# nameofuser1/vad

Hardware: AMD Instinct MI355X
Metric: MFCC+FFN frames/sec on 16 kHz 25 ms/10 ms hop (higher is better)
Workload: dtype f32; 1 GPU; C3/C4: MFCC + FFN VAD forward, 1 clip of F frames per GPU (25 ms frames, 10 ms hop, 512-pt FFT, 26 mel, 13 MFCC, analyser 5-frame features), labels gathered to rank 0; frames_per_gpu=1000000, ffn=13-64-64-2, hip_streams=2, parallelism=clip-shard x1

## Files before the change

### vad_amd/csrc/ffn_kernel.hip

```cpp
#include "vad_common.h"
#include "features.h"
#include "ffn_dev.h"

namespace vad {

enum Src { kFromMfcc = 0, kFromRows = 1 };

template <int KS0, int T1, int T2, int T3, int T4, int NC, int SRC>
__global__ __launch_bounds__(256) void ffn_kernel(FfnDev net, const float* __restrict__ in,
                                                  int64_t n_rows, int mfcc_n, int mode,
                                                  uint8_t* __restrict__ labels) {
  using TP = Topo<KS0, T1, T2, T3, T4, NC>;
  const int lane = threadIdx.x & 63;
  const int g = lane >> 4;
  const int jw = lane & 15;
  const int in_dim = net.dims[0];

  float fa[TP::NA];
  float fb[TP::NB];
  float fv[TP::NV + TP::NVB + 1];
  load_frags<TP>(net.frag, lane, fa, fb, fv);

  const int64_t n_tiles = (n_rows + 15) / 16;
  const int64_t wave_id = (int64_t)blockIdx.x * (blockDim.x >> 6) + (threadIdx.x >> 6);
  const int64_t n_waves = (int64_t)gridDim.x * (blockDim.x >> 6);
  for (int64_t tile = wave_id; tile < n_tiles; tile += n_waves) {
    const int64_t w = tile * 16 + jw;
    const bool valid = w < n_rows;
    float x[KS0];
#pragma unroll
    for (int s = 0; s < KS0; ++s) {
      const int f = 4 * s + g;
      float v = 0.f;
      if (f < in_dim && valid) {
        if constexpr (SRC == kFromMfcc) {
          const float* r0 = in + w * mfcc_n;
          v = window_feature(r0, r0 + mfcc_n, r0 + 2 * mfcc_n, r0 + 3 * mfcc_n, r0 + 4 * mfcc_n,
                             f, mfcc_n, mode);
        } else {
          v = in[w * in_dim + f];
        }
      }
      x[s] = v;
    }
    const f32x4 z = mlp_forward<KS0, T1, T2, T3, T4, NC>(fa, fb, fv, x);
    if (g == 0 && valid) {
      labels[w] = (uint8_t)argmax_classes(z, net.n_classes);
      store_logits(net.logits, w, z, net.n_classes);
    }
  }
}

#ifndef VAD_FFN_WIN_PRIO
#define VAD_FFN_WIN_PRIO 1
#endif
constexpr int kChunk = 64;
constexpr int kXStride = 68;

template <int KS0, int T1, int T2, int T3, int T4, int NC, int MN, bool H3, int MODE = -1>
__device__ __forceinline__ void ffn_window_body(const FfnDev& net, const float* __restrict__ mfcc,
                                                int64_t n_rows, int mfcc_n_rt, int mode_rt,
                                                uint8_t* __restrict__ labels) {
  const int mode = MODE >= 0 ? MODE : mode_rt;
  using TP = Topo<KS0, T1, T2, T3, T4, NC>;
  using HP = HTopo<TP, KS0, T1, T2, T3, T4>;
  static_assert(!H3 || (MN > 0 && MN * (kChunk / 4) <= 256), "split-f16 needs the sliding feature phase");
  __shared__ float rows[2][(kChunk + 4) * kMaxCoefs];
  __shared__ __attribute__((aligned(16))) float X[2][kChunk * kXStride];
  __shared__ int wnan[2][kChunk];
  const int mfcc_n = MN > 0 ? MN : mfcc_n_rt;
  const int tid = threadIdx.x;
  const int lane = tid & 63;
  const int wv = tid >> 6;
  const int g = lane >> 4;
  const int jw = lane & 15;
  const int in_dim = net.dims[0];
  const int nfeat = 3 * mfcc_n;

  constexpr int kNA = H3 ? 1 : TP::NA;
  constexpr int kNH = H3 ? HP::NS : 1;
  float fa[kNA];
  float fb[TP::NB];
  float fv[TP::NV + TP::NVB + 1];
  u4 fh[kNH][2];
  if constexpr (H3) {
    load_frags<TP, true>(net.frag, lane, fa, fb, fv);
    load_fragh<HP>(net.fragh, lane, fh);
    for (int i = tid; i < 2 * kChunk * kXStride; i += 256) (&X[0][0])[i] = 0.f;
  } else {
    load_frags<TP>(net.frag, lane, fa, fb, fv);
  }

  const int64_t n_frames = n_rows + 5;
  const int64_t n_chunks = (n_rows + kChunk - 1) / kChunk;
  constexpr int kRowRegs = ((kChunk + 4) * kMaxCoefs + 255) / 256;
  float pre[2][kRowRegs];
  constexpr int kPackRegs = MN > 0 ? ((kChunk + 4) * MN + 255) / 256 : 1;
  static_assert(MN == 0 || 256 * kPackRegs <= (kChunk + 4) * kMaxCoefs, "packed rows overflow");
  auto load_rows = [&](int64_t ch, float (&dst)[kRowRegs]) {
    const int64_t base = ch * kChunk;
    const int64_t avail = ch < n_chunks ? n_frames - base : 0;
    const int nr = (int)(avail < kChunk + 4 ? avail : kChunk + 4);
    if constexpr (MN > 0) {
#pragma unroll
      for (int q = 0; q < kPackRegs; ++q) {
        const int i = tid + 256 * q;
        const bool ok = i < nr * MN;
        const float v = mfcc[ok ? base * MN + i : 0];
        dst[q] = ok ? v : 0.f;
      }
    } else {
#pragma unroll
      for (int q = 0; q < kRowRegs; ++q) {
        const int i = tid + 256 * q;
        dst[q] = i < nr * mfcc_n ? mfcc[base * mfcc_n + i] : 0.f;
      }
    }
  };
  load_rows(blockIdx.x, pre[0]);
  load_rows(blockIdx.x + gridDim.x, pre[1]);
  int buf = 0;
  for (int64_t ch = blockIdx.x; ch < n_chunks; ch += gridDim.x, buf ^= 1) {
    const int64_t base = ch * kChunk;
    float* rw_ = rows[buf];
    float* Xb = X[buf];
    if constexpr (MN > 0) {
#pragma unroll
      for (int q = 0; q < kPackRegs; ++q) {
        rw_[tid + 256 * q] = pre[0][q];
        pre[0][q] = pre[1][q];
      }
    } else {
#pragma unroll
      for (int q = 0; q < kRowRegs; ++q) {
        const int i = tid + 256 * q;
        if (i < (kChunk + 4) * mfcc_n) {
          const int r = i / mfcc_n, c = i - r * mfcc_n;
          rw_[r * kMaxCoefs + c] = pre[0][q];
        }
        pre[0][q] = pre[1][q];
      }
    }
    if (H3 && tid < kChunk) wnan[buf][tid] = 0;
    __syncthreads();
    load_rows(ch + 2 * (int64_t)gridDim.x, pre[1]);
    const int64_t nwin64 = n_rows - base;
    const int nwin = (int)(nwin64 < kChunk ? nwin64 : kChunk);
    if constexpr (MN > 0 && MN * (kChunk / 4) <= 256) {
      const int c = tid % MN, q = tid / MN;
      if (q < kChunk / 4) {
        float a[8];
#pragma unroll
        for (int k = 0; k < 8; ++k) a[k] = rw_[(4 * q + k) * MN + c];
        const bool m0 = !H3 || c < in_dim, m1 = !H3 || MN + c < in_dim, m2 = !H3 || 2 * MN + c < in_dim;
        constexpr bool kD1 = !H3 || MN < 4 * KS0, kD2 = !H3 || 2 * MN < 4 * KS0;
#pragma unroll
        for (int k = 0; k < 4; ++k) {
          const Feat3 ft = feature_triple(a[k], a[k + 1], a[k + 2], a[k + 3], a[k + 4], mode);
          float* xw = Xb + (4 * q + k) * kXStride;
          if constexpr (H3) {
            const bool nan = (m0 || (kD2 && m2)) && ft.mn != ft.mn;
            __hip_atomic_fetch_or(&wnan[buf][4 * q + k], (int)nan, __ATOMIC_RELAXED,
                                  __HIP_MEMORY_SCOPE_WORKGROUP);
            xw[c] = m0 && !nan ? ft.mn : 0.f;
            if constexpr (kD1) xw[MN + c] = m1 ? ft.d1 : 0.f;
            if constexpr (kD2) xw[2 * MN + c] = m2 && !nan ? ft.d2 : 0.f;
          } else {
            xw[c] = ft.mn;
            xw[MN + c] = ft.d1;
            xw[2 * MN + c] = ft.d2;
          }
        }
      }
    } else
    for (int i = tid; i < nwin * mfcc_n; i += 256) {
      const int w = i / mfcc_n, c = i - w * mfcc_n;
      constexpr int kRS = MN > 0 ? MN : kMaxCoefs;
      const float* r = rw_ + w * kRS + c;
      const Feat3 ft = feature_triple(r[0], r[kRS], r[2 * kRS], r[3 * kRS], r[4 * kRS], mode);
      float* xw = Xb + w * kXStride;
      if constexpr (H3) {
        xw[c] = c < in_dim ? ft.mn : 0.f;
        xw[mfcc_n + c] = mfcc_n + c < in_dim ? ft.d1 : 0.f;
        xw[2 * mfcc_n + c] = 2 * mfcc_n + c < in_dim ? ft.d2 : 0.f;
      } else {
        xw[c] = ft.mn;
        xw[mfcc_n + c] = ft.d1;
        xw[2 * mfcc_n + c] = ft.d2;
      }
    }
    __syncthreads();
    const int wl = wv * 16 + jw;
    const int64_t w = base + wl;
#if VAD_FFN_WIN_PRIO
    __builtin_amdgcn_sched_barrier(0);
    __builtin_amdgcn_s_setprio(VAD_FFN_WIN_PRIO);
    __builtin_amdgcn_sched_barrier(0);
#endif
    f32x4 z;
    if constexpr (H3) {
      float x0[HP::K0][8];
      constexpr bool M0 = kMerge0<KS0>;
      const v4f* xr = reinterpret_cast<const v4f*>(Xb + wl * kXStride + 8 * (M0 ? (g & 1) : g));
#pragma unroll
      for (int s = 0; s < HP::K0; ++s) {
        const v4f lo4 = xr[8 * s], hi4 = xr[8 * s + 1];
#pragma unroll
        for (int q = 0; q < 4; ++q) {
          x0[s][q] = lo4[q];
          x0[s][q + 4] = hi4[q];
        }
      }
      if constexpr (M0) {
#pragma unroll
        for (int q = 0; q < 8; ++q)
          if (8 + q >= 13) x0[0][q] = 8 * (g & 1) + q < 13 ? x0[0][q] : 0.f;
      }
      z = mlp_forward_h3<KS0, T1, T2, T3, T4, NC>(FragRegs{fh}, (const float*)fb, (const float*)fv, x0);
      if (wnan[buf][wl]) z = (f32x4){__builtin_nanf(""), __builtin_nanf(""), __builtin_nanf(""), __builtin_nanf("")};
    } else {
      float x[KS0];
#pragma unroll
      for (int s = 0; s < KS0; ++s) {
        const int f = 4 * s + g;
        x[s] = (f < in_dim && f < nfeat && wl < nwin) ? Xb[wl * kXStride + f] : 0.f;
      }
      z = mlp_forward<KS0, T1, T2, T3, T4, NC>(fa, fb, fv, x);
    }
#if VAD_FFN_WIN_PRIO
    __builtin_amdgcn_sched_barrier(0);
    __builtin_amdgcn_s_setprio(0);
    __builtin_amdgcn_sched_barrier(0);
#endif
    if (g == 0 && wl < nwin) {
      labels[w] = (uint8_t)argmax_classes(z, net.n_classes);
      store_logits(net.logits, w, z, net.n_classes);
    }
  }
}

template <int KS0, int T1, int T2, int T3, int T4, int NC, int MN>
__global__ __launch_bounds__(256) void ffn_window_kernel(FfnDev net, const float* __restrict__ mfcc,
                                                         int64_t n_rows, int mfcc_n_rt, int mode,
                                                         uint8_t* __restrict__ labels) {
  ffn_window_body<KS0, T1, T2, T3, T4, NC, MN, false>(net, mfcc, n_rows, mfcc_n_rt, mode, labels);
}

template <int KS0, int T1, int T2, int T3, int T4, int NC, int MN, int MODE>
__global__ __launch_bounds__(256) __attribute__((amdgpu_waves_per_eu(2))) void ffn_window_h3_kernel(
    FfnDev net, const float* __restrict__ mfcc, int64_t n_rows, int mfcc_n_rt, int mode,
    uint8_t* __restrict__ labels) {
  ffn_window_body<KS0, T1, T2, T3, T4, NC, MN, true, MODE>(net, mfcc, n_rows, mfcc_n_rt, mode, labels);
}

#ifndef VAD_FFN_WAVE
#define VAD_FFN_WAVE 1
#endif
#ifndef VAD_FFN_PF
#define VAD_FFN_PF 2
#endif
#ifndef VAD_FFN_WAVE_MFMA_OUT
#define VAD_FFN_WAVE_MFMA_OUT 0
#endif
#ifndef VAD_FFN_LDS_SLOTS
#define VAD_FFN_LDS_SLOTS 1
#endif
#ifndef VAD_FFN_ALL_LDS
#define VAD_FFN_ALL_LDS 1
#endif
template <int KS0, int NC>
struct WaveResidency {
  static constexpr bool kAll = VAD_FFN_ALL_LDS != 0 && KS0 == 4 && NC <= 2;
  static constexpr bool kLdsFrags = KS0 == 10 || NC > 2 || kAll;
  static constexpr bool kLdsSlots = (VAD_FFN_LDS_SLOTS != 0 && !kLdsFrags) || kAll;
#ifndef VAD_FFN_ALL_WPS
#define VAD_FFN_ALL_WPS 4
#endif
  static constexpr int kWavesPerSimd = kAll ? VAD_FFN_ALL_WPS : KS0 == 10 ? 3 : kLdsSlots ? 3 : 2;
};
template <int LO_FROM>
struct FragSplitRes {
  const u4 (*p)[2];
  const u4* lo;
  int base;
  __device__ u4 get(int sl, int h) const {
    return (h == 1 && base + sl >= LO_FROM) ? lo[(base + sl - LO_FROM) * 64] : p[sl][h];
  }
  __device__ FragSplitRes at(int off) const { return {p + off, lo, base + off}; }
};
struct LdsRow {
  const float* p;
  __device__ float operator[](int s) const { return p[s]; }
  __device__ LdsRow operator+(int off) const { return {p + off}; }
};
constexpr int kWRows = (kWTile + 4) * 13;
constexpr int kWRowRegs = (kWRows + 63) / 64;

#ifndef VAD_FFN_WPB
#define VAD_FFN_WPB 4
#endif
constexpr int kWpb = VAD_FFN_WPB;
template <int KS0, int T1, int T2, int T3, int T4, int NC, int MODE, bool LG>
__global__ __launch_bounds__(64 * kWpb) __attribute__((amdgpu_waves_per_eu(WaveResidency<KS0, NC>::kWavesPerSimd))) void ffn_wave_kernel(
    FfnDev net, const float* __restrict__ mfcc, int64_t n_rows, uint8_t* __restrict__ labels) {
  using TP = Topo<KS0, T1, T2, T3, T4, NC, VAD_FFN_WAVE_MFMA_OUT != 0>;
  using HP = HTopo<TP, KS0, T1, T2, T3, T4>;
  constexpr int MN = 13;
  static_assert(KS0 == 4 || KS0 == 10, "specialised topologies: 13 or 39 inputs");
  constexpr int IN = KS0 == 4 ? MN : 3 * MN;
  constexpr int XS = 32 * HP::K0 + 4;
  __shared__ float rows_s[kWpb][kWRows];
  __shared__ __attribute__((aligned(16))) float x_s[kWpb][kWTile * XS];
  __shared__ int flat_s[kWpb][kWTile];
  const int lane = threadIdx.x & 63;
  const int wv = __builtin_amdgcn_readfirstlane(threadIdx.x >> 6);
  const int g = lane >> 4;
  const int jw = lane & 15;
  float* R = rows_s[wv];
  float* X = x_s[wv];
  int* FL = flat_s[wv];

  constexpr bool kLdsFrags = WaveResidency<KS0, NC>::kLdsFrags;
  constexpr bool kLdsSlots = WaveResidency<KS0, NC>::kLdsSlots;
  constexpr int NSL = TP::NB + TP::NV + TP::NVB;
  constexpr bool kDiff = NC == 2 && TP::VL && TP::NL == 3 && kLdsSlots;
  constexpr int NSD = kDiff ? TP::TIL * 4 + 1 : 0;
  constexpr int NSLP = (NSL + NSD + 3) & ~3;
  __shared__ __attribute__((aligned(16))) float slot_s[kLdsSlots ? 4 * NSLP : 1];
#ifndef VAD_FFN_PRIO
#define VAD_FFN_PRIO 3
#endif
#ifndef VAD_FFN_PRIO_FEAT
#define VAD_FFN_PRIO_FEAT 0
#endif
#ifndef VAD_FFN_LO_ALL
#define VAD_FFN_LO_ALL 1
#endif
  constexpr int kLoFrom = VAD_FFN_LO_ALL ? 0 : HP::S0;
  constexpr int kLoSlots = kLdsSlots && !kLdsFrags ? HP::NS - kLoFrom : 0;
  __shared__ u4 fhlo_s[kLoSlots > 0 ? kLoSlots * 64 : 1];
  float fa[1];
  float fb[kLdsSlots ? 1 : TP::NB];
  float fv[kLdsSlots ? 1 : TP::NV + TP::NVB + 1];
  if constexpr (kLdsSlots) {
    auto slot_val = [&](int sl, int gg) {
      const int src_sl = sl < TP::NB ? TP::NA_ALL + sl
                                     : TP::NA_ALL + TP::NB + (sl - TP::NB < TP::NV ? sl - TP::NB
                                                                                  : 4 * TP::TIL * 4 + sl - TP::NB - TP::NV);
      return net.frag[src_sl * 64 + 16 * gg];
    };
    for (int i = threadIdx.x; i < 4 * NSLP; i += 64 * kWpb) {
      const int gg = i / NSLP, sl = i - gg * NSLP;
      float v = 0.f;
      if (sl < NSL) {
        v = slot_val(sl, gg);
      } else if (sl < NSL + NSD) {
        const int q = sl - NSL;
        v = q < TP::TIL * 4 ? slot_val(TP::NB + TP::TIL * 4 + q, gg) - slot_val(TP::NB + q, gg)
                            : slot_val(TP::NB + TP::NV + 1, gg) - slot_val(TP::NB + TP::NV, gg);
      }
      slot_s[i] = v;
    }
    for (int i = threadIdx.x; i < kLoSlots * 64; i += 64 * kWpb)
      fhlo_s[i] = reinterpret_cast<const u4*>(net.fragh)[(2 * (kLoFrom + i / 64) + 1) * 64 + (i & 63)];
    __syncthreads();
  } else {
    load_frags<TP, true>(net.frag, lane, fa, fb, fv);
  }
  const auto fbs = [&] {
    if constexpr (kLdsSlots) return LdsRow{slot_s + g * NSLP};
    else return (const float*)fb;
  }();
  const auto fvs = [&] {
    if constexpr (kLdsSlots) return LdsRow{slot_s + g * NSLP + TP::NB};
    else return (const float*)fv;
  }();
  __shared__ u4 fh_s[kLdsFrags ? HP::NS * 2 * 64 : 1];
  u4 fh_r[kLdsFrags ? 1 : HP::NS][2];
  if constexpr (kLdsFrags) {
    for (int i = threadIdx.x; i < HP::NS * 2 * 64; i += 64 * kWpb) fh_s[i] = reinterpret_cast<const u4*>(net.fragh)[i];
    __syncthreads();
  } else {
    load_fragh<HP>(net.fragh, lane, *reinterpret_cast<u4(*)[HP::NS][2]>(fh_r));
  }
  const auto fh = [&] {
    if constexpr (kLdsFrags) return FragLds{fh_s, lane};
    else if constexpr (kLdsSlots) return FragSplitRes<kLoFrom>{fh_r, fhlo_s + lane, 0};
    else return FragRegs{fh_r};
  }();
  for (int i = lane; i < kWTile * XS; i += 64) X[i] = 0.f;

  const int64_t n_tiles = (n_rows + kWTile - 1) / kWTile;
  const int64_t total = (n_rows + 4) * MN;
  const int64_t wave_id = (int64_t)blockIdx.x * kWpb + wv;
  const int64_t n_waves = (int64_t)gridDim.x * kWpb;
  auto load = [&](int64_t t, float (&dst)[kWRowRegs]) {
    const int64_t base = t * (kWTile * MN);
    const float* tb = mfcc + base;
    const int64_t rem = total - 1 - base;
    const unsigned limb = 4u * (unsigned)(rem < kWRows ? rem : kWRows);
#pragma unroll
    for (int q = 0; q < kWRowRegs; ++q) {
      const unsigned ob = 4u * (unsigned)(lane + 64 * q);
      dst[q] = *reinterpret_cast<const float*>(reinterpret_cast<const char*>(tb) + (ob < limb ? ob : limb));
    }
  };
  __builtin_amdgcn_s_waitcnt(0x0f70);
  auto tile_body = [&](int64_t t, int64_t tn, float (&pre)[kWRowRegs]) {
    wave_lds_handoff();
#pragma unroll
    for (int q = 0; q < kWRowRegs; ++q)
      if (lane + 64 * q < kWRows) R[lane + 64 * q] = pre[q];
    load(tn < n_tiles ? tn : t, pre);
#if VAD_FFN_PRIO_FEAT
    __builtin_amdgcn_sched_barrier(0);
    __builtin_amdgcn_s_setprio(VAD_FFN_PRIO_FEAT);
    __builtin_amdgcn_sched_barrier(0);
#endif
    wave_tile_features<IN, XS, MODE>(R, X, FL, lane);
#if VAD_FFN_PRIO || VAD_FFN_PRIO_FEAT
    __builtin_amdgcn_sched_barrier(0);
    __builtin_amdgcn_s_setprio(VAD_FFN_PRIO);
    __builtin_amdgcn_sched_barrier(0);
#endif
    f32x4 z;
    int lab;
    if constexpr (kDiff) {
      lab = wave_tile_label2<KS0, T1, T2, IN, XS, false, wave_tile_in_bounded<MODE, IN>>(
          X, FL, lane, fh, fbs, fvs, LdsRow{slot_s + g * NSLP + NSL}, net.h1_bounded, LG ? &z : nullptr);
    } else {
      lab = wave_tile_classify<KS0, T1, T2, T3, T4, NC, VAD_FFN_WAVE_MFMA_OUT != 0, IN, XS, false,
                               wave_tile_in_bounded<MODE, IN>>(X, FL, lane, fh, fbs, fvs, net.n_classes, z);
    }
#if VAD_FFN_PRIO && !VAD_FFN_PRIO_FEAT
    __builtin_amdgcn_sched_barrier(0);
    __builtin_amdgcn_s_setprio(0);
    __builtin_amdgcn_sched_barrier(0);
#endif
    const int64_t w = t * kWTile + jw;
    if (g == 0 && w < n_rows) {
      labels[w] = (uint8_t)lab;
      if constexpr (LG) store_logits(net.logits, w, z, net.n_classes);
    }
  };
#ifndef VAD_FFN_PF_ALL
#define VAD_FFN_PF_ALL 1
#endif
  constexpr int kPF = WaveResidency<KS0, NC>::kAll ? VAD_FFN_PF_ALL : VAD_FFN_PF;
  float pre[kPF][kWRowRegs];
#pragma unroll
  for (int k = 0; k < kPF; ++k) {
    const int64_t tk = wave_id + k * n_waves;
    load(tk < n_tiles ? tk : 0, pre[k]);
  }
  for (int64_t t = wave_id; t < n_tiles; t += kPF * n_waves) {
#pragma unroll
    for (int k = 0; k < kPF; ++k) {
      const int64_t tk = t + k * n_waves;
      if (k > 0 && tk >= n_tiles) break;
      tile_body(tk, tk + kPF * n_waves, pre[k]);
    }
  }
}

#ifndef VAD_FFN_GROUP
#define VAD_FFN_GROUP 2
#endif
#ifndef VAD_FFN_GROUP_WPS
#define VAD_FFN_GROUP_WPS 0
#endif
template <int NT>
constexpr int kGroupWps = VAD_FFN_GROUP_WPS ? VAD_FFN_GROUP_WPS : NT <= 2 ? 4 : 2;
#ifndef VAD_FFN_GROUP_WPB
#define VAD_FFN_GROUP_WPB 8
#endif
constexpr int kGWpb = VAD_FFN_GROUP_WPB;
template <int MODE, int NT>
__global__ __launch_bounds__(64 * kGWpb) __attribute__((amdgpu_waves_per_eu(kGroupWps<NT>))) void ffn_wave_group_kernel(
    FfnDev net, const float* __restrict__ mfcc, int64_t n_rows, uint8_t* __restrict__ labels) {
  constexpr int KS0 = 4, T1 = 4, T2 = 4, NC = 2, MN = 13, IN = 13, XS = 20;
  using TP = Topo<KS0, T1, T2, 1, 0, NC, false>;
  using HP = HTopo<TP, KS0, T1, T2, 1, 0>;
  static_assert(TP::VL && TP::NL == 3, "VALU output layer");
  __shared__ float rows_s[kGWpb][NT][kWRows];
  __shared__ __attribute__((aligned(16))) float x_s[kGWpb][NT][kWTile * XS];
  __shared__ int flat_s[kGWpb][NT][kWTile];
  constexpr int NSL = TP::NB + TP::NV + TP::NVB;
  constexpr int NSD = TP::TIL * 4 + 1;
  constexpr int NSLP = (NSL + NSD + 3) & ~3;
  __shared__ __attribute__((aligned(16))) float slot_s[4 * NSLP];
  __shared__ u4 fh_s[HP::NS * 2 * 64];
  const int lane = threadIdx.x & 63;
  const int wv = __builtin_amdgcn_readfirstlane(threadIdx.x >> 6);
  const int g = lane >> 4;
  const int jw = lane & 15;
  const int64_t n_tiles = (n_rows + kWTile - 1) / kWTile;
  const int64_t total = (n_rows + 4) * MN;
  const int64_t wave_id = (int64_t)blockIdx.x * kGWpb + wv;
  const int64_t n_waves = (int64_t)gridDim.x * kGWpb;
  auto load = [&](int64_t t, float (&dst)[kWRowRegs]) {
    const int64_t base = t * (kWTile * MN);
    const float* tb = mfcc + base;
    const int64_t rem = total - 1 - base;
    const unsigned limb = 4u * (unsigned)(rem < kWRows ? rem : kWRows);
#pragma unroll
    for (int q = 0; q < kWRowRegs; ++q) {
      const unsigned ob = 4u * (unsigned)(lane + 64 * q);
      dst[q] = *reinterpret_cast<const float*>(reinterpret_cast<const char*>(tb) + (ob < limb ? ob : limb));
    }
  };
  auto member = [&](int64_t t, int k) { return t + k * n_waves < n_tiles ? t + k * n_waves : t; };
  float pre[NT][kWRowRegs];
  if (wave_id < n_tiles) {
#pragma unroll
    for (int k = 0; k < NT; ++k) load(member(wave_id, k), pre[k]);
  }
  {
    auto slot_val = [&](int sl, int gg) {
      const int src_sl = sl < TP::NB ? TP::NA_ALL + sl
                                     : TP::NA_ALL + TP::NB + (sl - TP::NB < TP::NV ? sl - TP::NB
                                                                                  : 4 * TP::TIL * 4 + sl - TP::NB - TP::NV);
      return net.frag[src_sl * 64 + 16 * gg];
    };
    for (int i = threadIdx.x; i < 4 * NSLP; i += 64 * kGWpb) {
      const int gg = i / NSLP, sl = i - gg * NSLP;
      float v = 0.f;
      if (sl < NSL) {
        v = slot_val(sl, gg);
      } else if (sl < NSL + NSD) {
        const int q = sl - NSL;
        v = q < TP::TIL * 4 ? slot_val(TP::NB + TP::TIL * 4 + q, gg) - slot_val(TP::NB + q, gg)
                            : slot_val(TP::NB + TP::NV + 1, gg) - slot_val(TP::NB + TP::NV, gg);
      }
      slot_s[i] = v;
    }
    for (int i = threadIdx.x; i < HP::NS * 2 * 64; i += 64 * kGWpb) fh_s[i] = reinterpret_cast<const u4*>(net.fragh)[i];
    __syncthreads();
  }
  const LdsRow fbs{slot_s + g * NSLP};
  const LdsRow fvs{slot_s + g * NSLP + TP::NB};
  const LdsRow fds{slot_s + g * NSLP + NSL};
  const FragLds fh{fh_s, lane};
  for (int k = 0; k < NT; ++k)
    for (int i = lane; i < kWTile * XS; i += 64) x_s[wv][k][i] = 0.f;

  __builtin_amdgcn_s_waitcnt(0x0f70);
  for (int64_t t = wave_id; t < n_tiles; t += NT * n_waves) {
    const int64_t tn = t + NT * n_waves < n_tiles ? t + NT * n_waves : t;
    wave_lds_handoff();
#pragma unroll
    for (int k = 0; k < NT; ++k)
#pragma unroll
      for (int q = 0; q < kWRowRegs; ++q)
        if (lane + 64 * q < kWRows) rows_s[wv][k][lane + 64 * q] = pre[k][q];
#pragma unroll
    for (int k = 0; k < NT; ++k) load(member(tn, k), pre[k]);
    wave_tile_features<IN, XS, MODE, NT, kWRows - kWTile * MN>(rows_s[wv][0], x_s[wv][0], flat_s[wv][0], lane);
#if VAD_FFN_PRIO
    __builtin_amdgcn_sched_barrier(0);
    __builtin_amdgcn_s_setprio(VAD_FFN_PRIO);
    __builtin_amdgcn_sched_barrier(0);
#endif
    float x[NT][1][8];
    int fl[NT];
#pragma unroll
    for (int k = 0; k < NT; ++k) fl[k] = wave_tile_operands<1, IN, XS, false>(x_s[wv][k], flat_s[wv][k], lane, x[k]);
    f32x4 h[NT][T2];
    mlp_hidden2_h3_multi<KS0, T1, T2, NT>(fh, fbs, x, h);
    int lab[NT];
#pragma unroll
    for (int k = 0; k < NT; ++k) lab[k] = valu_label2<TP, T2>(fds, fvs, h[k], fl[k]);
#if VAD_FFN_PRIO
    __builtin_amdgcn_sched_barrier(0);
    __builtin_amdgcn_s_setprio(0);
    __builtin_amdgcn_sched_barrier(0);
#endif
#pragma unroll
    for (int k = 0; k < NT; ++k) {
      const int64_t tk = member(t, k);
      const int64_t w = tk * kWTile + jw;
      if (g == 0 && (k == 0 || tk != t) && w < n_rows) labels[w] = (uint8_t)lab[k];
    }
  }
}

template <int KS0, int T1, int T2, int T3, int T4, int NC>
__global__ __launch_bounds__(256) void stream_ffn_kernel(FfnDev net, const float* __restrict__ newrow,
                                                         float* __restrict__ ring,
                                                         int* __restrict__ count, int64_t n_streams,
                                                         int mfcc_n, uint8_t* __restrict__ labels) {
  using TP = Topo<KS0, T1, T2, T3, T4, NC>;
  const int lane = threadIdx.x & 63;
  const int g = lane >> 4;
  const int jw = lane & 15;
  const int in_dim = net.dims[0];
  float fa[TP::NA];
  float fb[TP::NB];
  float fv[TP::NV + TP::NVB + 1];
  load_frags<TP>(net.frag, lane, fa, fb, fv);

  const int64_t n_tiles = (n_streams + 15) / 16;
  const int64_t wave_id = (int64_t)blockIdx.x * (blockDim.x >> 6) + (threadIdx.x >> 6);
  const int64_t n_waves = (int64_t)gridDim.x * (blockDim.x >> 6);
  for (int64_t tile = wave_id; tile < n_tiles; tile += n_waves) {
    const int64_t s = tile * 16 + jw;
    const bool valid = s < n_streams;
    const int c = valid ? count[s] : 0;
    const bool have = valid && c >= 5;
    float* rs = ring + s * 5 * mfcc_n;
    float x[KS0];
#pragma unroll
    for (int k = 0; k < KS0; ++k) {
      const int f = 4 * k + g;
      float v = 0.f;
      if (have && f < in_dim) {
        v = window_feature(rs + ((c + 0) % 5) * mfcc_n, rs + ((c + 1) % 5) * mfcc_n,
                           rs + ((c + 2) % 5) * mfcc_n, rs + ((c + 3) % 5) * mfcc_n,
                           rs + ((c + 4) % 5) * mfcc_n, f, mfcc_n, VAD_FEAT_ANALYSER);
      }
      x[k] = v;
    }
    const f32x4 z = mlp_forward<KS0, T1, T2, T3, T4, NC>(fa, fb, fv, x);
    if (valid) {
      if (g == 0) labels[s] = have ? (uint8_t)argmax_classes(z, net.n_classes) : (uint8_t)255;
      float* dst = rs + (c % 5) * mfcc_n;
      for (int cc = g; cc < mfcc_n; cc += 4) dst[cc] = newrow[s * mfcc_n + cc];
      if (g == 0) count[s] = (c + 1 >= 10) ? c + 1 - 5 : c + 1;
    }
  }
}

__global__ __launch_bounds__(256) void features_kernel(const float* __restrict__ mfcc,
                                                       int64_t n_rows, int mfcc_n, int mode,
                                                       float* __restrict__ out) {
  const int nf = 3 * mfcc_n;
  const int64_t total = n_rows * nf;
  for (int64_t i = (int64_t)blockIdx.x * blockDim.x + threadIdx.x; i < total;
       i += (int64_t)gridDim.x * blockDim.x) {
    const int64_t w = i / nf;
    const int f = (int)(i - w * nf);
    const float* r0 = mfcc + w * mfcc_n;
    out[i] = window_feature(r0, r0 + mfcc_n, r0 + 2 * mfcc_n, r0 + 3 * mfcc_n, r0 + 4 * mfcc_n, f,
                            mfcc_n, mode);
  }
}

template <int KS0, int T1, int T2, int T3, int T4, int NC = 4>
static hipError_t launch_stream_topo(const FfnDev& net, const float* newrow, float* ring, int* count,
                                     int64_t n_streams, int mfcc_n, uint8_t* labels, hipStream_t st) {
  const int64_t n_tiles = (n_streams + 15) / 16;
  int64_t blocks = (n_tiles + 3) / 4;
  if (blocks > 2048) blocks = 2048;
  hipLaunchKernelGGL((stream_ffn_kernel<KS0, T1, T2, T3, T4, NC>), dim3((int)blocks), dim3(256), 0, st,
                     net, newrow, ring, count, n_streams, mfcc_n, labels);
  return hipGetLastError();
}

static int ffn_num_cus() {
  static int n = 0;
  if (n == 0) {
    int dev = 0;
    if (hipGetDevice(&dev) != hipSuccess ||
        hipDeviceGetAttribute(&n, hipDeviceAttributeMultiprocessorCount, dev) != hipSuccess || n <= 0)
      n = 256;
  }
  return n;
}

template <int KS0, int T1, int T2, int T3, int T4, int NC = 4>
static hipError_t launch_topo(const FfnDev& net, int src, const float* in, int64_t n_rows,
                              int mfcc_n, int mode, uint8_t* labels, hipStream_t st) {
  const int64_t n_tiles = (n_rows + 15) / 16;
  int64_t blocks = (n_tiles + 3) / 4;
  if (blocks > 2048) blocks = 2048;
  if (src == kFromMfcc) {
    int64_t chunks = (n_rows + kChunk - 1) / kChunk;
    const int64_t cap = 2 * ffn_num_cus();
    if (chunks > cap) chunks = cap;
    constexpr bool kH3 = (KS0 == 10 && T1 == 4 && T2 == 2 && T3 == 1 && T4 == 1) ||
                         (KS0 == 4 && T1 == 4 && T2 == 4 && T3 == 1 && T4 == 0);
    if constexpr (kH3) {
      if constexpr (KS0 == 4 && NC <= 2) {
        if (VAD_FFN_GROUP >= 2 && mfcc_n == 13 && net.fragh && !net.logits && net.h1_bounded &&
            mode == VAD_FEAT_ANALYSER && net.n_classes == 2) {
          constexpr int NT = VAD_FFN_GROUP >= 2 ? VAD_FFN_GROUP : 2;
          const int64_t n_tiles = (n_rows + kWTile - 1) / kWTile;
          int64_t gblocks = ((n_tiles + NT - 1) / NT + kGWpb - 1) / kGWpb;
          const int64_t gcap = kGroupWps<NT> * 4 / kGWpb * ffn_num_cus();
          if (gblocks > gcap) gblocks = gcap;
          hipLaunchKernelGGL((ffn_wave_group_kernel<VAD_FEAT_ANALYSER, NT>), dim3((int)gblocks), dim3(64 * kGWpb), 0, st,
                             net, in, n_rows, labels);
          return hipGetLastError();
        }
      }
      if (mfcc_n == 13 && net.fragh && VAD_FFN_WAVE) {
        int64_t wblocks = (n_rows + kWpb * kWTile - 1) / (kWpb * kWTile);
        const int64_t wcap = WaveResidency<KS0, NC>::kWavesPerSimd * 4 / kWpb * ffn_num_cus();
        if (wblocks > wcap) wblocks = wcap;
        const dim3 grid((int)wblocks), blk(64 * kWpb);
        if (mode == VAD_FEAT_OFFLINE) {
          if (net.logits)
            hipLaunchKernelGGL((ffn_wave_kernel<KS0, T1, T2, T3, T4, NC, VAD_FEAT_OFFLINE, true>), grid, blk, 0, st,
                               net, in, n_rows, labels);
          else
            hipLaunchKernelGGL((ffn_wave_kernel<KS0, T1, T2, T3, T4, NC, VAD_FEAT_OFFLINE, false>), grid, blk, 0, st,
                               net, in, n_rows, labels);
        } else {
          if (net.logits)
            hipLaunchKernelGGL((ffn_wave_kernel<KS0, T1, T2, T3, T4, NC, VAD_FEAT_ANALYSER, true>), grid, blk, 0, st,
                               net, in, n_rows, labels);
          else
            hipLaunchKernelGGL((ffn_wave_kernel<KS0, T1, T2, T3, T4, NC, VAD_FEAT_ANALYSER, false>), grid, blk, 0, st,
                               net, in, n_rows, labels);
        }
        return hipGetLastError();
      }
      if (mfcc_n == 13 && net.fragh) {
        if (mode == VAD_FEAT_OFFLINE)
          hipLaunchKernelGGL((ffn_window_h3_kernel<KS0, T1, T2, T3, T4, NC, 13, VAD_FEAT_OFFLINE>),
                             dim3((int)chunks), dim3(256), 0, st, net, in, n_rows, mfcc_n, mode, labels);
        else
          hipLaunchKernelGGL((ffn_window_h3_kernel<KS0, T1, T2, T3, T4, NC, 13, VAD_FEAT_ANALYSER>),
                             dim3((int)chunks), dim3(256), 0, st, net, in, n_rows, mfcc_n, mode, labels);
        return hipGetLastError();
      }
    }
    if (mfcc_n == 13)
      hipLaunchKernelGGL((ffn_window_kernel<KS0, T1, T2, T3, T4, NC, 13>), dim3((int)chunks), dim3(256), 0,
                         st, net, in, n_rows, mfcc_n, mode, labels);
    else
      hipLaunchKernelGGL((ffn_window_kernel<KS0, T1, T2, T3, T4, NC, 0>), dim3((int)chunks), dim3(256), 0,
                         st, net, in, n_rows, mfcc_n, mode, labels);
  } else
    hipLaunchKernelGGL((ffn_kernel<KS0, T1, T2, T3, T4, NC, kFromRows>), dim3((int)blocks), dim3(256), 0,
                       st, net, in, n_rows, mfcc_n, mode, labels);
  return hipGetLastError();
}

hipError_t launch_ffn(const FfnDev& net, int src, const float* in, int64_t n_rows, int mfcc_n,
                      int mode, uint8_t* labels, hipStream_t st) {
  if (n_rows <= 0) return hipSuccess;
  const int* t = net.tiles;
  if (net.n_layers == 4 && net.ks0 == 10 && t[0] == 4 && t[1] == 2 && t[2] == 1 && t[3] == 1)
    return launch_topo<10, 4, 2, 1, 1>(net, src, in, n_rows, mfcc_n, mode, labels, st);
  if (net.n_layers == 3 && net.ks0 == 4 && t[0] == 4 && t[1] == 4 && t[2] == 1) {
    if (net.n_classes <= 2)
      return launch_topo<4, 4, 4, 1, 0, 2>(net, src, in, n_rows, mfcc_n, mode, labels, st);
    return launch_topo<4, 4, 4, 1, 0>(net, src, in, n_rows, mfcc_n, mode, labels, st);
  }
  switch (net.n_layers) {
    case 1: return launch_topo<16, 1, 0, 0, 0>(net, src, in, n_rows, mfcc_n, mode, labels, st);
    case 2: return launch_topo<16, 4, 1, 0, 0>(net, src, in, n_rows, mfcc_n, mode, labels, st);
    case 3: return launch_topo<16, 4, 4, 1, 0>(net, src, in, n_rows, mfcc_n, mode, labels, st);
    default: return launch_topo<16, 4, 4, 4, 1>(net, src, in, n_rows, mfcc_n, mode, labels, st);
  }
}

hipError_t launch_stream_ffn(const FfnDev& net, const float* newrow, float* ring, int* count,
                             int64_t n_streams, int mfcc_n, uint8_t* labels, hipStream_t st) {
  if (n_streams <= 0) return hipSuccess;
  const int* t = net.tiles;
  if (net.n_layers == 4 && net.ks0 == 10 && t[0] == 4 && t[1] == 2 && t[2] == 1 && t[3] == 1)
    return launch_stream_topo<10, 4, 2, 1, 1>(net, newrow, ring, count, n_streams, mfcc_n, labels, st);
  if (net.n_layers == 3 && net.ks0 == 4 && t[0] == 4 && t[1] == 4 && t[2] == 1) {
    if (net.n_classes <= 2)
      return launch_stream_topo<4, 4, 4, 1, 0, 2>(net, newrow, ring, count, n_streams, mfcc_n, labels, st);
    return launch_stream_topo<4, 4, 4, 1, 0>(net, newrow, ring, count, n_streams, mfcc_n, labels, st);
  }
  switch (net.n_layers) {
    case 1: return launch_stream_topo<16, 1, 0, 0, 0>(net, newrow, ring, count, n_streams, mfcc_n, labels, st);
    case 2: return launch_stream_topo<16, 4, 1, 0, 0>(net, newrow, ring, count, n_streams, mfcc_n, labels, st);
    case 3: return launch_stream_topo<16, 4, 4, 1, 0>(net, newrow, ring, count, n_streams, mfcc_n, labels, st);
    default: return launch_stream_topo<16, 4, 4, 4, 1>(net, newrow, ring, count, n_streams, mfcc_n, labels, st);
  }
}

hipError_t launch_features(const float* mfcc, int64_t n_rows, int mfcc_n, int mode, float* out,
                           hipStream_t st) {
  if (n_rows <= 0) return hipSuccess;
  int64_t blocks = (n_rows * 3 * mfcc_n + 255) / 256;
  if (blocks > 4096) blocks = 4096;
  hipLaunchKernelGGL(features_kernel, dim3((int)blocks), dim3(256), 0, st, mfcc, n_rows, mfcc_n,
                     mode, out);
  return hipGetLastError();
}

}
```

Measured before the change: 3.498 billion frames/s.

## Process adjacent tile pairs per wave with one contiguous buffer load

When the group size is 2, each wave now handles two adjacent tiles instead of two strided tiles. It loads their shared MFCC rows, overlap included, with one bounds-checked raw buffer load, and writes labels for both tiles with one contiguous per-lane store. Loop counters drop to 32-bit ints. The aim is to cut duplicate overlap loads, the clamped-address arithmetic, and scattered byte stores. In exchange it relies on feature extraction handling a contiguous 2-tile row window, and it adds an n_rows guard for the 32-bit indexing.

```diff
diff --git a/vad_amd/csrc/ffn_kernel.hip b/vad_amd/csrc/ffn_kernel.hip
--- a/vad_amd/csrc/ffn_kernel.hip
+++ b/vad_amd/csrc/ffn_kernel.hip
@@ -1,6 +1,8 @@
 #include "vad_common.h"
 #include "features.h"
 #include "ffn_dev.h"
+
+#include <type_traits>
 
 namespace vad {
 
@@ -466,6 +468,9 @@
 #ifndef VAD_FFN_GROUP
 #define VAD_FFN_GROUP 2
 #endif
+#ifndef VAD_FFN_PAIR_ADJ
+#define VAD_FFN_PAIR_ADJ 1
+#endif
 #ifndef VAD_FFN_GROUP_WPS
 #define VAD_FFN_GROUP_WPS 0
 #endif
@@ -482,7 +487,12 @@
   using TP = Topo<KS0, T1, T2, 1, 0, NC, false>;
   using HP = HTopo<TP, KS0, T1, T2, 1, 0>;
   static_assert(TP::VL && TP::NL == 3, "VALU output layer");
-  __shared__ float rows_s[kGWpb][NT][kWRows];
+  constexpr bool kAdj = VAD_FFN_PAIR_ADJ != 0 && NT == 2;
+  constexpr int kPairItems = 2 * kWTile * MN;
+  constexpr int kPairRows = (2 * kWTile + 4) * MN;
+  constexpr int kPairRegs = (kPairRows + 63) / 64;
+  constexpr int kRSlice = kAdj ? 64 * kPairRegs : NT * kWRows;
+  __shared__ float rows_s[kGWpb][kRSlice];
   __shared__ __attribute__((aligned(16))) float x_s[kGWpb][NT][kWTile * XS];
   __shared__ int flat_s[kGWpb][NT][kWTile];
   constexpr int NSL = TP::NB + TP::NV + TP::NVB;
@@ -511,7 +521,24 @@
   };
   auto member = [&](int64_t t, int k) { return t + k * n_waves < n_tiles ? t + k * n_waves : t; };
   float pre[NT][kWRowRegs];
-  if (wave_id < n_tiles) {
+  float prp[kPairRegs];
+  const int n_pairs = (int)((n_tiles + 1) / 2);
+  const int n_full = n_pairs - 2;
+  const int pstep = (int)n_waves;
+  const int lane4 = 4 * lane;
+  auto load_pair = [&](const float* tb, int p) {
+    const int left = p < n_full ? 64 * kPairRegs : p < n_pairs ? (int)(total - (int64_t)p * kPairItems) : 0;
+    const int nrec = 4 * (left < 64 * kPairRegs ? left : 64 * kPairRegs);
+    const __amdgpu_buffer_rsrc_t rs =
+        __builtin_amdgcn_make_buffer_rsrc(const_cast<float*>(tb), (short)0, nrec, 0x00020000);
+#pragma unroll
+    for (int q = 0; q < kPairRegs; ++q)
+      prp[q] = __builtin_bit_cast(float, __builtin_amdgcn_raw_buffer_load_b32(rs, lane4 + 256 * q, 0, 0));
+  };
+  const float* tb = mfcc + wave_id * kPairItems;
+  if constexpr (kAdj) {
+    load_pair(tb, wave_id < n_pairs ? (int)wave_id : n_pairs);
+  } else if (wave_id < n_tiles) {
 #pragma unroll
     for (int k = 0; k < NT; ++k) load(member(wave_id, k), pre[k]);
   }
@@ -545,17 +572,32 @@
     for (int i = lane; i < kWTile * XS; i += 64) x_s[wv][k][i] = 0.f;
 
   __builtin_amdgcn_s_waitcnt(0x0f70);
-  for (int64_t t = wave_id; t < n_tiles; t += NT * n_waves) {
-    const int64_t tn = t + NT * n_waves < n_tiles ? t + NT * n_waves : t;
+  using trip_t = std::conditional_t<kAdj, int, int64_t>;
+  const trip_t t_first = kAdj ? (trip_t)(wave_id < n_pairs ? wave_id : n_pairs) : (trip_t)wave_id;
+  const trip_t t_end = kAdj ? (trip_t)n_pairs : (trip_t)n_tiles;
+  const trip_t t_step = kAdj ? (trip_t)pstep : (trip_t)(NT * n_waves);
+  uint8_t* lb = labels + wave_id * (2 * kWTile);
+  int rlane = lane;
+  asm volatile("" : "+v"(rlane));
+  for (trip_t t = t_first; t < t_end; t += t_step) {
     wave_lds_handoff();
-#pragma unroll
-    for (int k = 0; k < NT; ++k)
-#pragma unroll
-      for (int q = 0; q < kWRowRegs; ++q)
-        if (lane + 64 * q < kWRows) rows_s[wv][k][lane + 64 * q] = pre[k][q];
-#pragma unroll
-    for (int k = 0; k < NT; ++k) load(member(tn, k), pre[k]);
-    wave_tile_features<IN, XS, MODE, NT, kWRows - kWTile * MN>(rows_s[wv][0], x_s[wv][0], flat_s[wv][0], lane);
+    if constexpr (kAdj) {
+#pragma unroll
+      for (int q = 0; q < kPairRegs; ++q) rows_s[wv][rlane + 64 * q] = prp[q];
+      tb += (int64_t)pstep * kPairItems;
+      load_pair(tb, t + pstep < n_pairs ? t + pstep : n_pairs);
+      wave_tile_features<IN, XS, MODE, NT, 0>(rows_s[wv], x_s[wv][0], flat_s[wv][0], lane);
+    } else {
+      const int64_t tn = t + NT * n_waves < n_tiles ? t + NT * n_waves : t;
+#pragma unroll
+      for (int k = 0; k < NT; ++k)
+#pragma unroll
+        for (int q = 0; q < kWRowRegs; ++q)
+          if (lane + 64 * q < kWRows) rows_s[wv][k * kWRows + lane + 64 * q] = pre[k][q];
+#pragma unroll
+      for (int k = 0; k < NT; ++k) load(member(tn, k), pre[k]);
+      wave_tile_features<IN, XS, MODE, NT, kWRows - kWTile * MN>(rows_s[wv], x_s[wv][0], flat_s[wv][0], lane);
+    }
 #if VAD_FFN_PRIO
     __builtin_amdgcn_sched_barrier(0);
     __builtin_amdgcn_s_setprio(VAD_FFN_PRIO);
@@ -575,11 +617,17 @@
     __builtin_amdgcn_s_setprio(0);
     __builtin_amdgcn_sched_barrier(0);
 #endif
-#pragma unroll
-    for (int k = 0; k < NT; ++k) {
-      const int64_t tk = member(t, k);
-      const int64_t w = tk * kWTile + jw;
-      if (g == 0 && (k == 0 || tk != t) && w < n_rows) labels[w] = (uint8_t)lab[k];
+    if constexpr (kAdj) {
+      const int nst = t < n_pairs - 1 ? 2 * kWTile : (int)(n_rows - (int64_t)t * (2 * kWTile));
+      if (lane < nst) lb[lane] = (uint8_t)(g == 0 ? lab[0] : lab[NT - 1]);
+      lb += (int64_t)pstep * (2 * kWTile);
+    } else {
+#pragma unroll
+      for (int k = 0; k < NT; ++k) {
+        const int64_t tk = member(t, k);
+        const int64_t w = tk * kWTile + jw;
+        if (g == 0 && (k == 0 || tk != t) && w < n_rows) labels[w] = (uint8_t)lab[k];
+      }
     }
   }
 }
@@ -682,7 +730,7 @@
     if constexpr (kH3) {
       if constexpr (KS0 == 4 && NC <= 2) {
         if (VAD_FFN_GROUP >= 2 && mfcc_n == 13 && net.fragh && !net.logits && net.h1_bounded &&
-            mode == VAD_FEAT_ANALYSER && net.n_classes == 2) {
+            mode == VAD_FEAT_ANALYSER && net.n_classes == 2 && n_rows < (int64_t(1) << 35)) {
           constexpr int NT = VAD_FFN_GROUP >= 2 ? VAD_FFN_GROUP : 2;
           const int64_t n_tiles = (n_rows + kWTile - 1) / kWTile;
           int64_t gblocks = ((n_tiles + NT - 1) / NT + kGWpb - 1) / kGWpb;
```

Result: no change. 3.528 billion frames/s, median of 6 (+0.9%).
